# FrozenBurning/SceneDreamer

Hardware: NVIDIA H100
Metric: rendered Msamples/sec at 960x540x24spp (higher is better)
Workload: dtype f16x3 split (f32-grade), f32 accumulate; table/compositing f32

## Files before the change

scenedreamer_b200/csrc/render_fused.cu:

```cuda
#include <stdlib.h>

#include <map>
#include <mutex>
#include <utility>

#include "rf_common.cuh"

namespace rf {

int32_t *g_debug_buffer = nullptr;

struct Sample { float depth, nd; int idx; };

__device__ __forceinline__ Sample sample_at(const Params &p, const float *st, int row, int k, const float *frac,
                                            long long ray) {
    const float total = st[kStTotal * kRows + row];
    float r0, r1;
    if (p.uniforms == nullptr) {
        r0 = __fmul_rn(frac[k], total);
        r1 = __fmul_rn(frac[k + 1], total);
    } else {
        const float ns = (float)(p.S + 1);
        const bool any = total > 0.0f;
        const float u0 = any ? __ldg(p.uniforms + ray * (p.S + 1) + k) : 0.0f;
// ... 180 lines not shown
            h[q] = __byte_perm(a, b, 0x7632);
            const float la = v[2 * q] - __uint_as_float(a & 0xFFFF0000u);
            const float lb = v[2 * q + 1] - __uint_as_float(b & 0xFFFF0000u);
            l[q] = tc05::pack2<true>(la, lb);
        }
    } else {
#pragma unroll
        for (int q = 0; q < 4; q++) { h[q] = tc05::pack2<false>(v[2 * q], v[2 * q + 1]); l[q] = 0; }
    }
    hi = make_uint4(h[0], h[1], h[2], h[3]);
    lo = make_uint4(l[0], l[1], l[2], l[3]);
}

template <int PREC> __device__ __forceinline__ uint32_t one16() { return PREC == 1 ? 0x3F80u : 0x3C00u; }

template <bool RAW5D, int GU, int PREC, class Rec>
__device__ __forceinline__ void encode_features(const Params &p, uint32_t mask, const float *sScale, int half, const float (&x)[5],
                                                bool oob, uint4 (&fh)[8], uint4 (&fl)[8], Rec &&rec) {
#pragma unroll
    for (int i = 0; i < 8; i++) {
        const int level = half + 2 * i;
        float res[8];
        if (oob) {
#pragma unroll
            for (int c = 0; c < 8; c++) res[c] = 0.0f;
        } else {
            encode_level<RAW5D, GU>(p.table + ((size_t)level << p.log2_T) * 8, mask, sScale[level], x, res);
        }
        split8<PREC>(res, fh[i], fl[i]);
        rec(level, res);
    }
}

__device__ __forceinline__ uint4 label_chunk(uint32_t label, int half, uint32_t one) {
    const int k = (int)label - 8 * half;
    const uint32_t v = (k >= 0 && k < 8) ? one << (16 * (k & 1)) : 0u, q = k >> 1;
    return make_uint4(q == 0 ? v : 0u, q == 1 ? v : 0u, q == 2 ? v : 0u, (q == 3 ? v : 0u) | (half == 1 ? one << 16 : 0u));
}

template <bool X3>
__device__ __forceinline__ void store_layer0(uint8_t *sHhi, uint8_t *sHlo, int row, int half, const uint4 (&fh)[8],
                                             const uint4 (&fl)[8], uint4 ext) {
#pragma unroll
    for (int i = 0; i < 8; i++) {
        const uint32_t off = tc05::chunk_off(kRows, row, half + 2 * i);
        *reinterpret_cast<uint4 *>(sHhi + off) = fh[i];
        if constexpr (X3) *reinterpret_cast<uint4 *>(sHlo + off) = fl[i];
    }
    const uint32_t off = tc05::chunk_off(kRows, row, kFeat / 8 + half);
    *reinterpret_cast<uint4 *>(sHhi + off) = ext;
    if constexpr (X3) *reinterpret_cast<uint4 *>(sHlo + off) = make_uint4(0, 0, 0, 0);
}

template <int PREC, bool RAW5D, int MODE, bool TRAIN, bool RAYQ = false, int GU = 8>
__global__ void __launch_bounds__(kThreads, 1)
mlp_kernel(const Params p)
{
    static_assert(!RAYQ || (MODE == kRender && !TRAIN && !RAW5D), "ray slots: inference render over the pre-blended table");
    constexpr bool SKY = MODE == kSky, BWD = MODE == kBwd || MODE == kSkyBwd, SKYBWD = MODE == kSkyBwd;
    constexpr bool ONE_STEP = SKY || SKYBWD;
    constexpr int NACT = Net<MODE>::NACT;
    static_assert(!TRAIN || ((MODE == kRender || MODE == kSky) && !RAW5D), "the training record is written by the forward networks");
    static_assert(!BWD || PREC == 1, "the gradient chains run in the range-safe bf16x3 mode");
    constexpr bool X3 = PREC != 0;
    constexpr bool BF16 = PREC == 1;
    constexpr Smem SM = smem_map();
    constexpr int PARTS = X3 ? 2 : 1;
    constexpr int NH = Net<MODE>::NH, NL = Net<MODE>::NL;
    static_assert(SM.total <= 232448, "shared memory map exceeds the 227 KB a CTA can have");
    static_assert(Net<MODE>::NBIAS <= Net<kRender>::NBIAS, "bias table slot");
    extern __shared__ __align__(1024) uint8_t smem[];
    uint8_t *sHhi = smem + SM.h_hi;
    uint8_t *sHlo = smem + SM.h_lo;
    uint8_t *sRing = smem + SM.ring;
    float *sF = reinterpret_cast<float *>(smem + SM.fsec);
    float *sBias = reinterpret_cast<float *>(smem + SM.bias);
    float *sScale = reinterpret_cast<float *>(smem + SM.scales);
    float *sFrac = reinterpret_cast<float *>(smem + SM.frac);
    float *sSig = reinterpret_cast<float *>(smem + SM.sig);
    float *sState = reinterpret_cast<float *>(smem + SM.state);
    uint64_t *bars = reinterpret_cast<uint64_t *>(smem + SM.bars);
    uint32_t *sWalk = reinterpret_cast<uint32_t *>(smem + SM.walk);
    constexpr uint32_t kSlot = 16384, kSlabB = 2048 * PARTS;
    constexpr int kSps = kSlot / kSlabB;
    constexpr int kStepStages = step_stages<MODE>(kSps);
    constexpr uint32_t kWalk0 = hand_plan<MODE>(0).walk, kWalkH = hand_plan<MODE>(1).walk, kWalkL = hand_plan<MODE>(NL - 1).walk;
    constexpr uint32_t kSrc0 = hand_plan<MODE>(0).src, kSrcH = hand_plan<MODE>(1).src, kSrcL = hand_plan<MODE>(NL - 1).src;
    static_assert(SKYBWD || hand_all_staged<MODE>(NL - 1), "the epilogue reads the last layer from the operand buffer only");
    constexpr bool ESTOP = MODE == kRender && !TRAIN;
    volatile int *sStop = reinterpret_cast<volatile int *>(smem + SM.stop);
    volatile int *sVote = sStop + 2;
    int *sVoted = const_cast<int *>(sStop) + 4;

    const int tid = threadIdx.x, warp = tid >> 5, lane = tid & 31;
    const int wmult = (MODE == kBwd && p.work_mult > 1) ? p.work_mult : 1;
    const int n_work = RAYQ ? (int)gridDim.x : (ONE_STEP ? p.n_tiles : *p.n_live * wmult);
    auto rec_work = [&](int work) {
        if constexpr (MODE != kBwd) return work;
        int first;
        asm volatile("ld.global.nc.s32 %0, [%1];" : "=r"(first) : "l"(p.view));
        return work + first * wmult;
    };
    constexpr bool STATE = MODE == kRender;
    const int S = ONE_STEP ? 1 : p.S;
    const int SL = RAYQ ? 0x3fffffff : S;
    uint4 *sInfo = reinterpret_cast<uint4 *>(sState + kStFloats * kRows);
    int *sDone = reinterpret_cast<int *>(sInfo + 4 * kRows);
    int2 *sCur = reinterpret_cast<int2 *>(sDone + 2 * kRows);
    volatile int *sExh = reinterpret_cast<volatile int *>(sCur + kRows);
    static_assert(4 * kRows * 16 + 2 * kRows * 4 + kRows * 8 + 32 <= kStFloats * kRows * 4, "ray-slot bookkeeping fits the second state buffer");

    if (tid == 0) {
        for (int i = 0; i < 4; i++) tc05::mbar_init(&bars[B_WFULL + i], 1);
        tc05::mbar_init(&bars[B_FEAT], kGatherThreads);
        tc05::mbar_init(&bars[B_HFREE], 1);
        for (int rb = 0; rb < 2; rb++) {
            tc05::mbar_init(&bars[B_OPND + rb], kEpiThreads / 2);
            tc05::mbar_init(&bars[B_ACC + rb], 1);
            tc05::mbar_init(&bars[B_OUTRDY + rb], 1);
            tc05::mbar_init(&bars[B_EPIDONE + rb], kEpiThreads / 2);
            tc05::mbar_init(&bars[B_EPIDONE + 2 + rb], kEpiThreads / 2);
        }
        for (int i = 0; i < 2; i++) { tc05::mbar_init(&bars[B_STRDY + i], kRows); tc05::mbar_init(&bars[B_STFREE + i], kEpiThreads); }
        tc05::mbar_init(&bars[B_COMP], kEpiThreads);
        for (int i = 0; i < 4; i++) tc05::mbar_init(&bars[B_WEMPTY + i], 4);
        tc05::fence_mbar_init();
        int k = 0;
        for (int l = 0; l < NL; l++) {
            const int nK = layerK<MODE>(l) / 16, ncb = layerN<MODE>(l) / 64, nsb = block_stages(nK, kSps);
            const uint32_t walk = l == 0 ? kWalk0 : (l == NL - 1 ? kWalkL : kWalkH);
            for (int rb = 0; rb < 2; rb++)
                for (int pos = 0; pos < ncb; pos++) {
                    const int c = (walk >> (8 * pos)) & 3u;
                    uint32_t po = (uint32_t)(layerOff<MODE>(l, PARTS) + (int64_t)c * nK * kSlabB);
                    for (int js = 0; js < nsb; js++) {
                        const uint32_t bytes = (uint32_t)stage_slabs(nK, kSps, js) * kSlabB;
                        sWalk[k++] = (po >> 11) | ((bytes >> 11) << 16);
                        po += bytes;
                    }
                }
        }
    }
    if (tid < 2) { sStop[tid] = RAYQ ? 0x7fffffff : kMaxS + 1; sVote[tid] = 0; sVoted[tid] = 0; }
    if constexpr (RAYQ) {
        for (int i = tid; i < kRows; i += kThreads) { sCur[i] = make_int2(-1, 0); sDone[i] = 0; sDone[kRows + i] = 0; }
        if (tid < 5) sExh[tid] = 0;
    }
    volatile int *sWork = reinterpret_cast<volatile int *>(smem + SM.sched);
    volatile int *sPub = sWork + 4;
    if (tid == 0) *sPub = 0;
    const bool dyn = STATE && !RAYQ && p.work_counter != nullptr;
    auto fetch_work = [&](int it) -> int {
        if (!dyn) {
            const int w = (int)blockIdx.x + it * (int)gridDim.x;
            return w < n_work ? w : -1;
        }
        while (*sPub <= it) {
        }
        return sWork[it & 3];
    };
    if (STATE) {
        for (int i = tid; i < kLevels; i += kThreads) sScale[i] = exp2f(i * p.level_S) * p.base_res - 1.0f;
        for (int i = tid; i <= p.S; i += kThreads) sFrac[i] = p.fractions[i];
    }
    __syncthreads();
    const uint32_t mask = SKY ? 0u : ((1u << p.log2_T) - 1u);

    if (warp < 8) {
        set_maxnreg<kRegsEpi>();
        const int row = tid & (kRows - 1), half = tid >> 7;
        const int rb = row >> 6;
        const bool rb_lead = (tid & 191) == 0;
        auto last_vote = [&](int s) {
            __threadfence_block();
            const bool last = atomicAdd(&sVoted[s & 1], 1) == 1;
            if (last) {
                sVoted[s & 1] = 0;
                __threadfence_block();
            }
            return last;
        };
        const float *acc_cta = p.acc + (size_t)blockIdx.x * 2 * kRows * kAccCols;
        uint32_t n = 0;
        int loaded_img = -1;
        for (int it = 0;; it++) {
            const int work = fetch_work(it);
            if (work < 0) break;
            const int tile = RAYQ ? 0 : (ONE_STEP ? work : p.tile_list[rec_work(work) / wmult]);
            const TileCoord tc = tile_coord(p, tile);
            const int buf = it & 1;
            const float *st = sState + buf * kStFloats * kRows;
            if (Net<MODE>::TAIL && loaded_img != tc.img) {
                const float *packF = reinterpret_cast<const float *>(p.pack + (long long)tc.img * p.pack_stride +
                                                                     layerOff<MODE>(NL, PARTS));
                asm volatile("bar.sync 1, 256;" ::: "memory");
                for (int i = tid; i < kFTotal; i += kEpiThreads) sF[i] = __ldg(packF + i);
                asm volatile("bar.sync 1, 256;" ::: "memory");
                loaded_img = tc.img;
            }
            const int y = tc.y0 + (row >> 4), x = tc.x0 + (row & 15);
            const bool in_img = (y < p.H) && (x < p.W);
            const long long ray = ((long long)tc.img * p.H + y) * p.W + x;
            uint32_t flags = in_img ? 4u : 0u, labs = 0;
            float dir0 = 0.0f, ori0 = 0.0f;
            if (STATE && !RAYQ) {
                tc05::mbar_wait(&bars[B_STRDY + buf], (it >> 1) & 1);
                flags = __float_as_uint(st[kStFlags * kRows + row]);
                labs = __float_as_uint(st[kStLab * kRows + row]);
                dir0 = st[(kStDir + 0) * kRows + row];
                ori0 = __ldg(p.cam_ori + tc.img * 3);
            }
            (void)labs;
            const bool live = flags & 1u, valid = flags & 4u;
            float outc[32];
#pragma unroll
            for (int c = 0; c < 32; c++) outc[c] = 0.0f;
            float Wsum = 0.0f, Dsum = 0.0f, Dcomp = 0.0f, Eexcl = 0.0f;
            bool is_gnd = false;
// ... 132 lines not shown
                stg_ld<32>(sHhi, sHlo, row, ccol, c);
                if constexpr (BWD) {
                    float c2[32];
                    stg_ld<32>(sHhi, sHlo, row, ccol + 32, c2);
                    tc05::mbar_arrive(&bars[B_EPIDONE + (go & 1u) * 2 + rb]);
                    if (rb_lead) SDB_STAMP(n, NH, 5 + 2 * rb);
                    float *dst = p.tr.dx0 + slot * kFeat + half * 64;
#pragma unroll
                    for (int q = 0; q < 4; q++) st_global_v8f(dst + 8 * q, &c[8 * q]);
#pragma unroll
                    for (int q = 0; q < 4; q++) st_global_v8f(dst + 32 + 8 * q, &c2[8 * q]);
                    continue;
                }
                tc05::mbar_arrive(&bars[B_EPIDONE + (go & 1u) * 2 + rb]);
                if (rb_lead) SDB_STAMP(n, NH, 5 + 2 * rb);
                if constexpr (SKY) {
#pragma unroll
                    for (int j = 0; j < 32; j++) outc[j] = c[j];
                } else if constexpr (RAYQ) {
                    tc05::named_sync(4 + rb, 128);
                    const float sigma = (sSig[row] + sSig[kRows + row]) + sF[kFBsig];
                    const uint4 info = sInfo[(s & 3) * kRows + row];
                    const int rq = (int)info.z;
                    const uint32_t code = info.w;
                    const int s_ray = (int)(code & 0xffu);
                    const bool act = rq >= 0 && rq != skip_ray;
                    if (act && (code & 0x100u)) {
#pragma unroll
                        for (int j = 0; j < 32; j++) outc[j] = 0.0f;
                        Wsum = 0.0f; Dsum = 0.0f; Dcomp = 0.0f; Eexcl = 0.0f;
                    }
                    float w = 0.0f;
                    bool fin = false;
                    if (act) {
                        const float depth = __uint_as_float(info.x), nd = __uint_as_float(info.y);
                        w = sample_weight(sigma, nd, p.dists_scale, Eexcl);
                        composite_add(w, depth, Wsum, Dsum, Dcomp);
                        if (half == 0 && p.weights_out) p.weights_out[(long long)rq * S + s_ray] = w;
                        fin = (code & 0x200u) || (p.early_T > 0.0f && expf(-Eexcl) < p.early_T);
                    }
                    colour_add(w, c, outc);
                    if (act && fin) {
                        const bool nosky = !(code & 0x800u) || (code & 0x1000u);
                        finish_ray(p, 0, rq, nosky, half * 32, outc, Wsum, __fadd_rn(Dsum, Dcomp), half == 0);
                        skip_ray = (code & 0x200u) ? -1 : rq;
                    }
                    if (half == 0) sDone[(s & 1) * kRows + row] = (act && fin && !(code & 0x200u)) ? rq + 1 : 0;
                    {
                        const bool idle = !act || fin;
                        const bool wall = __all_sync(0xffffffffu, idle);
                        if (lane == 0 && !wall) sVote[s & 1] = 1;
                        tc05::named_sync(4 + rb, 128);
                        if (rb_lead && last_vote(s)) {
                            if (sVote[s & 1] == 0 && sExh[s & 3] != 0 && sStop[0] > s + 2) sStop[0] = s + 2;
                            sVote[s & 1] = 0;
                        }
                    }
                    tc05::mbar_arrive(&bars[B_COMP]);
                } else {
                    tc05::named_sync(4 + rb, 128);
                    const float sigma = (sSig[row] + sSig[kRows + row]) + sF[kFBsig];
                    float w = sample_weight(sigma, sm.nd, p.dists_scale, Eexcl);
                    w = live ? w : 0.0f;
                    composite_add(w, sm.depth, Wsum, Dsum, Dcomp);
                    if constexpr (TRAIN) {
                        if (half == 0) { p.tr.sig[slot] = sigma; p.tr.nds[slot] = __fmul_rn(sm.nd, p.dists_scale); }
                        float *cd = p.tr.c + slot * kOutC + half * 32;
#pragma unroll
                        for (int q = 0; q < 4; q++) st_global_v8f(cd + 8 * q, &c[8 * q]);
                    }
                    if (half == 0 && valid) {
                        if (p.weights_out) p.weights_out[ray * S + s] = w;
                        if (p.rdepth_out) p.rdepth_out[ray * S + s] = sm.depth;
                    }
                    if (ESTOP && p.early_T > 0.0f) {
                        const bool done = !live || expf(-Eexcl) < p.early_T;
                        const bool wall = __all_sync(0xffffffffu, done);
                        if (lane == 0 && !wall) sVote[s & 1] = 1;
                        tc05::named_sync(4 + rb, 128);
                        if (rb_lead && last_vote(s)) {
                            if (sVote[s & 1] == 0 && sStop[buf] > S) sStop[buf] = s + 2;
                            sVote[s & 1] = 0;
                        }
                    }
                    colour_add(w, c, outc);
                }
            }
            if constexpr (SKY) {
                if (valid) {
                    float4 *dst = reinterpret_cast<float4 *>(p.sky_out + ray * kOutC + half * 32);
#pragma unroll
                    for (int q = 0; q < 8; q++) dst[q] = make_float4(outc[4 * q], outc[4 * q + 1], outc[4 * q + 2], outc[4 * q + 3]);
                }
                float *red = sSig;
                asm volatile("bar.sync 1, 256;" ::: "memory");
#pragma unroll
                for (int j = 0; j < 32; j++) {
                    float v = valid ? outc[j] : 0.0f;
#pragma unroll
                    for (int o = 16; o > 0; o >>= 1) v += __shfl_xor_sync(0xffffffffu, v, o);
                    if (lane == 0) red[(warp & 3) * kOutC + half * 32 + j] = v;
                }
                asm volatile("bar.sync 1, 256;" ::: "memory");
                if (tid < kOutC)
                    p.sky_partial[(long long)tile * kOutC + tid] =
                        (red[tid] + red[kOutC + tid]) + (red[2 * kOutC + tid] + red[3 * kOutC + tid]);
            } else if constexpr (RAYQ) {
// ... 41 lines not shown
          }
          for (int s = 0; s < SL; s++, n++) {
              if (ESTOP && s >= 2 && s >= sStop[it & 1]) break;
#pragma unroll 1
              for (int l = 0; l < NL; l++) {
                  const uint32_t g = n * NL + l, buf = g & 1u;
                  const int N = layerN<MODE>(l), nK = layerK<MODE>(l) / 16;
                  const int ncb = N / 64, nsb = block_stages(nK, kSps), ns0 = group0_stages(nK, kSps);
#pragma unroll 1
                  for (int rb = 0; rb < 2; rb++) {
                      if (t == 0) SDB_MARK(2, 1, n, l);
                      if (g >= 2) tc05::mbar_wait(&bars[B_EPIDONE + buf * 2 + rb], ((g >> 1) - 1) & 1);
                      if (l == 0) {
                          if (rb == 0) tc05::mbar_wait(&bars[B_FEAT], n & 1);
                      } else {
                          tc05::mbar_wait(&bars[B_OPND + rb], (n * NH + l - 1) & 1);
                      }
                      if (t == 0) SDB_MARK(2, 2, n, l);
                      if (t == 0) SDB_STAMP(n, l, 2 * rb);
                      TSplit ts;
                      ts.start();
                      const uint32_t dst = (blockIdx.x * 2 + buf) * kRows * kAccCols + acc_off(rb * 64, 0);
                      const uint32_t walk = l == 0 ? kWalk0 : (l == NL - 1 ? kWalkL : kWalkH);
                      float x[32], y[32];
                      auto issue = [&](float (&d)[32], int js0, int js1) {
                          for (int js = js0; js < js1; js++) {
                              const uint32_t slot = q & 3u;
                              tc05::mbar_wait(&bars[B_WFULL + slot], (q >> 2) & 1u);
                              ts.lap(kSplitFull);
                              const uint32_t sb = tc05::smem_u32(sRing + slot * kSlot);
                              const int kk0 = stage_slab0(nK, kSps, js), ns = stage_slabs(nK, kSps, js);
                              tc05::wgmma_fence();
#pragma unroll
                              for (int i = 0; i < kSps; i++) {
                                  if (i >= ns) break;
                                  const uint32_t aoff = (uint32_t)(kk0 + i) * 2 * kLboA + rb * 1024;
                                  const uint64_t ah = tc05::make_smem_desc(tc05::smem_u32(sHhi) + aoff, kLboA, kSbo);
                                  const uint64_t bh = tc05::make_smem_desc(sb + i * kSlabB, 1024, kSbo);
                                  tc05::wgmma_m64n64k16<BF16, 0, 0>(d, ah, bh, (js > js0 || i > 0) ? 1u : 0u);
                                  if constexpr (X3) {
                                      const uint64_t al = tc05::make_smem_desc(tc05::smem_u32(sHlo) + aoff, kLboA, kSbo);
                                      tc05::wgmma_m64n64k16<BF16, 0, 0>(d, al, bh, 1u);
                                      tc05::wgmma_m64n64k16<BF16, 0, 0>(d, ah, bh + (2048 >> 4), 1u);
                                  }
                              }
                              tc05::wgmma_commit();
                              q++;
                              ts.lap(kSplitIssue);
                          }
                      };
                      auto retire = [&](int pending) {
                          auto release = [&]() {
                              ts.lap(kSplitWait);
                              if (lane == 0) tc05::mbar_arrive(&bars[B_WEMPTY + (qr & 3u)]);
                              qr++;
                              ts.lap(kSplitRelease);
                          };
#pragma unroll 1
                          for (int k = pending - 1; k > 0; k--) {
                              tc05::wgmma_wait_n(k);
                              release();
                          }
                          tc05::wgmma_wait<0>();
                          if (pending > 0) release();
                      };
                      bool g0_done = false;
                      auto block = [&](float (&a)[32], float (&b)[32], int pos) {
                          const uint32_t w = walk >> (8 * pos);
                          const int c = (int)(w & 3u);
                          issue(b, ns0, nsb);
                          retire(g0_done ? nsb - ns0 : nsb);
                          g0_done = false;
                          tc05::wgmma_fence_acc(a);
                          tc05::wgmma_fence_acc(b);
                          if (nsb > ns0) {
#pragma unroll
                              for (int i = 0; i < 32; i++) a[i] = __fadd_rn(a[i], b[i]);
                          }
                          uint32_t ft;
                          asm volatile("mov.u32 %0, %%tid.x;" : "=r"(ft));
                          ft -= kMmaWarp0 * 32;
                          if (BIAS && l > 0) {
                              const float *bias = sBias + (l - 1) * kHidden + c * 64;
#pragma unroll
                              for (int i = 0; i < 32; i += 2) {
                                  const float2 bb = *reinterpret_cast<const float2 *>(bias + tc05::frag_col(ft, i));
                                  a[i] = __fadd_rn(a[i], bb.x);
                                  a[i + 1] = __fadd_rn(a[i + 1], bb.y);
                              }
                          }
                          ts.lap(kSplitReduce);
                          if (pos + 1 < ncb) issue(b, 0, ns0);
                          if (!(w & kHStaged)) {
#ifndef SDB_AB_NO_ACC
                              float *out = p.acc + (dst + (uint32_t)(c & 1) * 4096u + acc_off(tc05::frag_row(ft, 0), tc05::frag_col(ft, 0)));
#pragma unroll
                              for (int i = 0; i < 32; i += 2)
                                  *reinterpret_cast<float2 *>(out + (i >> 2) * 128 + ((i >> 1) & 1) * 32) = make_float2(a[i], a[i + 1]);
#endif
                          } else {
                              if (w & kHDelayed) {
                                  retire(ns0);
                                  g0_done = true;
                              }
                              if (l == 0 && (w & kHFirst) && g >= 1)
                                  tc05::mbar_wait(&bars[B_EPIDONE + ((g - 1) & 1u) * 2 + rb], ((g - 1) >> 1) & 1u);
                              if (w & kHBarrier) tc05::named_sync(3, 128);
// ... 207 lines not shown
                if (half == 0) {
                    const RayVoxels vox = ray_state(p, st, row, tc.img, pix, valid);
                    const uint32_t flags = (valid && vox.first != 0 ? 1u : 0u) | (vox.last == 0 ? 2u : 0u) | (valid ? 4u : 0u);
                    st[kStFlags * kRows + row] = __uint_as_float(flags);
                }
                asm volatile("bar.sync 2, 256;" ::: "memory");
                if (half == 0) tc05::mbar_arrive(&bars[B_STRDY + buf]);
                const bool live = __float_as_uint(st[kStFlags * kRows + row]) & 1u;
                const uint32_t labs = __float_as_uint(st[kStLab * kRows + row]);
                const float dir[3] = {st[(kStDir + 0) * kRows + row], st[(kStDir + 1) * kRows + row], st[(kStDir + 2) * kRows + row]};
                const float ori[3] = {__ldg(p.cam_ori + tc.img * 3 + 0), __ldg(p.cam_ori + tc.img * 3 + 1), __ldg(p.cam_ori + tc.img * 3 + 2)};
                float x5[5];
                x5[3] = __fmul_rn(__fadd_rn(__ldg(p.genc + tc.img * 2 + 0), 1.0f), 0.5f);
                x5[4] = __fmul_rn(__fadd_rn(__ldg(p.genc + tc.img * 2 + 1), 1.0f), 0.5f);

                for (int s = 0; s < S; s++, n++) {
                    uint4 fh[8], fl[8];
                    const Sample sm = sample_at(p, st, row, s, sFrac, ray);
                    const bool outside = grid_coord(p, dir, ori, sm.depth, x5);
                    const bool oob = !live || outside;
                    const uint32_t label = (labs >> (4 * sm.idx)) & 15u;
                    if constexpr (TRAIN) {
                        const long long slot = ((long long)work * S + s) * kRows + row;
                        if (half == 0) p.tr.x3[slot] = make_float4(x5[0], x5[1], x5[2], oob ? -1.0f : 1.0f);
                        *reinterpret_cast<uint4 *>(rec_chunk(p.tr.x0, slot, kX0Cols / 8, kFeat / 8 + half)) = label_chunk(label, half, one16<1>());
                    }
                    encode_features<RAW5D, 8, PREC>(p, mask, sScale, half, x5, oob, fh, fl, [&](int level, const float (&res)[8]) {
                        if constexpr (TRAIN) {
                            const long long slot = ((long long)work * S + s) * kRows + row;
                            *reinterpret_cast<uint4 *>(rec_chunk(p.tr.x0, slot, kX0Cols / 8, level)) =
                                make_uint4(tc05::pack2<true>(res[0], res[1]), tc05::pack2<true>(res[2], res[3]),
                                           tc05::pack2<true>(res[4], res[5]), tc05::pack2<true>(res[6], res[7]));
                        }
                    });
                    const uint4 ext = label_chunk(label, half, one16<PREC>());
                    if (gt == 0) SDB_MARK(4, 3, n, it);
                    if (n > 0) tc05::mbar_wait_backoff(&bars[B_HFREE], (n - 1) & 1);
                    if (gt == 0) SDB_MARK(4, 4, n, it);
                    if (ESTOP && s >= 2 && s >= sStop[buf]) break;
                    store_layer0<X3>(sHhi, sHlo, row, half, fh, fl, ext);
                    tc05::fence_proxy_async_smem();
                    tc05::mbar_arrive(&bars[B_FEAT]);
                }
            }
        }
    } else {
        set_maxnreg<kRegsProd>();
        if (warp == kProducerWarp0 && elect_one()) {
            uint32_t n = 0, q = 0;
            uint32_t waited = 0;
            auto wait_empty = [&]() {
                if (q < 4) return;
                const uint32_t c = SDB_CLOCK();
                tc05::mbar_wait(&bars[B_WEMPTY + (q & 3u)], ((q >> 2) - 1) & 1u);
                waited += SDB_CLOCK() - c;
            };
            for (int it = 0;; it++) {
                const int work = fetch_work(it);
                if (work < 0) break;
                const int tile = RAYQ ? 0 : (ONE_STEP ? work : p.tile_list[rec_work(work) / wmult]);
                const uint8_t *pack = p.pack + (long long)tile_coord(p, tile).img * p.pack_stride;
                for (int s = 0; s < SL; s++, n++) {
                    SDB_MARK(3, 1, n, it);
                    waited = 0;
                    wait_empty();
                    if (ESTOP && s >= 2 && s >= sStop[it & 1]) break;
                    for (int k = 0; k < kStepStages; k++, q++) {
                        if (k > 0) wait_empty();
                        const uint32_t e = sWalk[k], bytes = (e >> 16) << 11, slot = q & 3u;
                        tc05::mbar_arrive_expect_tx(&bars[B_WFULL + slot], bytes);
                        tc05::bulk_g2s(sRing + slot * kSlot, pack + ((e & 0xffffu) << 11), bytes, &bars[B_WFULL + slot]);
                    }
                    SDB_STAMP_PROD(n, waited);
                }
            }
        }
    }
}

__device__ __forceinline__ void sky_only_ray(const Params &p, int img, long long ray) {
    const bool is_gnd = __ldg(p.cam_ori + img * 3) <= 1.0f;
    const float none[kOutC] = {};
    finish_ray(p, img, ray, is_gnd, 0, none, 0.0f, 0.0f, true);
    for (int s = 0; s < p.S; s++) {
        if (p.weights_out) p.weights_out[ray * p.S + s] = 0.0f;
        if (p.rdepth_out) p.rdepth_out[ray * p.S + s] = 0.0f;
    }
}

__global__ void __launch_bounds__(kRows)
prepass_kernel(const Params p, int32_t *tile_list, int32_t *n_live)
{
    const int tile = blockIdx.x, row = threadIdx.x;
    const TileCoord tc = tile_coord(p, tile);
    const int y = tc.y0 + (row >> 4), x = tc.x0 + (row & 15);
    const bool valid = (y < p.H) && (x < p.W);
    const long long ray = ((long long)tc.img * p.H + y) * p.W + x;
    const bool live = valid && (__ldg(p.voxel_id + ray * p.M) != 0);
    const int any = __syncthreads_or(live ? 1 : 0);
    if (any) {
        if (row == 0) {
            const int w = atomicAdd(n_live, 1);
            tile_list[w] = tile;
            if (p.tr.tile_work) p.tr.tile_work[tile] = w;
        }
        return;
    }
    if (row == 0 && p.tr.tile_work) p.tr.tile_work[tile] = -1;
    if (valid) sky_only_ray(p, tc.img, ray);
}

__global__ void __launch_bounds__(kRows)
train_prepass_kernel(const Params p, int32_t *hdr)
{
    const int tile = blockIdx.x, row = threadIdx.x;
    const TileCoord tc = tile_coord(p, tile);
    const int y = tc.y0 + (row >> 4), x = tc.x0 + (row & 15);
    const bool valid = (y < p.H) && (x < p.W);
    const long long ray = ((long long)tc.img * p.H + y) * p.W + x;
    const bool live = valid && (__ldg(p.voxel_id + ray * p.M) != 0);
    if (__syncthreads_or(live ? 1 : 0)) {
        if (row == 0) p.tr.tile_work[tile] = atomicAdd(hdr + 2 + 2 * tc.img, 1);
        return;
    }
    if (row == 0) p.tr.tile_work[tile] = -1;
    if (valid) sky_only_ray(p, tc.img, ray);
}

__global__ void __launch_bounds__(256)
train_list_kernel(const Params p, int32_t *hdr, int32_t *tile_list)
// ... 158 lines not shown
            float *F = reinterpret_cast<float *>(pack + layerOff<MODE>(NL, PARTS));
            float v = 0.0f;
            if (u < kHidden) v = wsig[u];
            else if (u == kFBsig) v = bsig[0];
            F[u] = v;
            return;
        }
        u -= kFTotal;
    }
    if (u >= Net<MODE>::NBIAS) return;
    const int l = 1 + (int)(u / kHidden), nn = (int)(u % kHidden);
    const float v = l == NL - 1 ? bout[nn] : bh[(long long)(l - 1) * kHidden + nn];
    reinterpret_cast<float *>(pack + biasOff<MODE>(PARTS))[u] = packed_value<PREC>(v);
}

template <bool SKY>
int launch_pack(const float *w0, const float *b0, const float *emb, int n_labels, const float *wh, const float *bh,
                const float *wsig, const float *bsig, const float *wout, const float *bout, int precision, void *pack,
                cudaStream_t st) {
    constexpr int MODE = SKY ? kSky : kRender;
    long long n = (SKY ? 0 : kFTotal) + Net<MODE>::NBIAS;
    for (int l = 0; l < Net<MODE>::NL; l++) n += (long long)layerK<MODE>(l) * layerN<MODE>(l);
    const int blocks = (int)((n + 255) / 256);
    if (precision == 1)
        pack_kernel<1, SKY><<<blocks, 256, 0, st>>>(w0, b0, emb, n_labels, wh, bh, wsig, bsig, wout, bout, (uint8_t *)pack);
    else if (precision == 2)
        pack_kernel<2, SKY><<<blocks, 256, 0, st>>>(w0, b0, emb, n_labels, wh, bh, wsig, bsig, wout, bout, (uint8_t *)pack);
    else
        pack_kernel<0, SKY><<<blocks, 256, 0, st>>>(w0, b0, emb, n_labels, wh, bh, wsig, bsig, wout, bout, (uint8_t *)pack);
    SDB_CHECK_LAUNCH();
    return SDB_OK;
}

static int acc_buffers(int grid, cudaStream_t st, float **out) {
    static std::mutex mu;
    static std::map<std::pair<int, cudaStream_t>, std::pair<float *, int>> bufs;
    int dev = 0;
    SDB_CUDA(cudaGetDevice(&dev));
    std::lock_guard<std::mutex> lk(mu);
    std::pair<float *, int> &b = bufs[std::make_pair(dev, st)];
    if (b.second < grid) {
        cudaStreamCaptureStatus cs = cudaStreamCaptureStatusNone;
        SDB_CUDA(cudaStreamIsCapturing(st, &cs));
        if (cs != cudaStreamCaptureStatusNone) return SDB_EUNSUPPORTED;
        if (b.first) SDB_CUDA(cudaFree(b.first));
        b = std::make_pair((float *)nullptr, 0);
        SDB_CUDA(cudaMalloc(&b.first, (size_t)grid * 2 * kRows * kAccCols * sizeof(float)));
        b.second = grid;
    }
    *out = b.first;
    return SDB_OK;
}

template <int PREC, bool RAW5D, int MODE, bool TRAIN = false, bool RAYQ = false, int GU = 8>
int launch_mlp(const Params &p_in, int grid, cudaStream_t st) {
    Params p = p_in;
    const int e = acc_buffers(grid, st, &p.acc);
    if (e != SDB_OK) return e;
    const size_t smem = smem_map().total;
    cudaFuncAttributes fa;
    SDB_CUDA(cudaFuncGetAttributes(&fa, mlp_kernel<PREC, RAW5D, MODE, TRAIN, RAYQ, GU>));
    if (fa.numRegs < kRegsLaunch) return SDB_EUNSUPPORTED;
    SDB_CUDA(cudaFuncSetAttribute(mlp_kernel<PREC, RAW5D, MODE, TRAIN, RAYQ, GU>, cudaFuncAttributeMaxDynamicSharedMemorySize, (int)smem));
    mlp_kernel<PREC, RAW5D, MODE, TRAIN, RAYQ, GU><<<grid, kThreads, smem, st>>>(p);
    SDB_CHECK_LAUNCH();
    return SDB_OK;
}

int launch_train_forward(const Params &p, int precision, int grid, cudaStream_t st) {
    return precision == 0 ? launch_mlp<0, false, kRender, true>(p, grid, st) : launch_mlp<2, false, kRender, true>(p, grid, st);
}
int launch_bwd_chain(const Params &p, int grid, cudaStream_t st) { return launch_mlp<1, false, kBwd>(p, grid, st); }
int launch_sky_train_forward(const Params &p, int grid, cudaStream_t st) { return launch_mlp<2, false, kSky, true>(p, grid, st); }
int launch_sky_bwd_chain(const Params &p, int grid, cudaStream_t st) { return launch_mlp<1, false, kSkyBwd>(p, grid, st); }
int launch_train_prepass(const Params &p, int32_t *hdr, int32_t *tile_list, cudaStream_t st) {
    SDB_CUDA(cudaMemsetAsync(hdr, 0, (size_t)(1 + 2 * p.n_img) * 4, st));
    train_prepass_kernel<<<p.n_tiles, kRows, 0, st>>>(p, hdr);
    SDB_CHECK_LAUNCH();
    train_list_kernel<<<(p.n_tiles + 255) / 256, 256, 0, st>>>(p, hdr, tile_list);
    SDB_CHECK_LAUNCH();
    return SDB_OK;
}
int launch_prepass(const Params &p, int32_t *ws, cudaStream_t st) {
    SDB_CUDA(cudaMemsetAsync(ws, 0, 16, st));
    prepass_kernel<<<p.n_tiles, kRows, 0, st>>>(p, ws + 4, ws);
    SDB_CHECK_LAUNCH();
    return SDB_OK;
}

template <int MODE>
__global__ void __launch_bounds__(256)
pack_bwd_kernel(const float *w1, const float *wh, const float *wsig, const float *wout, uint8_t *pack)
{
    constexpr int PARTS = 2, NL = Net<MODE>::NL;
    const long long t = blockIdx.x * (long long)blockDim.x + threadIdx.x;
    long long nW = 0;
    for (int l = 0; l < NL; l++) nW += (long long)layerK<MODE>(l) * layerN<MODE>(l);
    if (t < nW) {
        long long r = t;
        int l = 0;
        while (r >= (long long)layerK<MODE>(l) * layerN<MODE>(l)) { r -= (long long)layerK<MODE>(l) * layerN<MODE>(l); l++; }
        const int K = layerK<MODE>(l);
        const int nn = (int)(r / K), k = (int)(r % K);
        float v;
        if (l == 0) v = wout[(long long)k * kHidden + nn];
        else if (MODE == kBwd && l == NL - 1) v = w1[(long long)k * kFeat + nn];
        else v = wh[((long long)((MODE == kBwd ? 5 : 4) - l) * kHidden + k) * kHidden + nn];
        uint8_t *base = pack + layerOff<MODE>(l, PARTS);
        const __nv_bfloat16 hi = __float2bfloat16_rn(v);
        const __nv_bfloat16 lo = __float2bfloat16_rn(v - __bfloat162float(hi));
        *reinterpret_cast<__nv_bfloat16 *>(base + wpack_off(K / 16, PARTS, nn, k, 0)) = hi;
        *reinterpret_cast<__nv_bfloat16 *>(base + wpack_off(K / 16, PARTS, nn, k, 1)) = lo;
        return;
    }
    if (!Net<MODE>::TAIL) return;
    const long long u = t - nW;
    if (u >= kFTotal) return;
    float *F = reinterpret_cast<float *>(pack + layerOff<MODE>(NL, PARTS));
    F[u] = u < kHidden ? wsig[u] : 0.0f;
// ... 168 lines not shown
    p.sample_depth = sp->sample_depth; p.dists_scale = sp->dists_scale;
    p.early_T = sp->early_stop_transmittance > 0.0f ? sp->early_stop_transmittance : 0.0f;
    p.fractions = sp->d_fractions; p.uniforms = sp->d_uniforms;
    p.lut = sp->d_label_lut; p.n_lut = sp->n_lut;
    p.raw5d = sp->d_table != nullptr;
    p.table = p.raw5d ? sp->d_table : sp->d_table3;
    p.log2_T = sp->log2_T; p.level_S = sp->level_S; p.base_res = sp->base_res;
    p.pack = (const uint8_t *)sp->d_mlp_pack; p.pack_stride = sp->mlp_pack_stride;
    p.sky = sp->d_sky; p.sky_avg = sp->d_sky_avg;
    p.net_out = sp->d_net_out; p.depth_out = sp->d_depth_out; p.total_weight = sp->d_total_weight;
    p.weights_out = sp->d_weights_out; p.rdepth_out = sp->d_rand_depth_out;
    p.debug = g_debug_buffer;
    p.tiles_x = sdb_div_up(p.W, kTileW); p.tiles_y = sdb_div_up(p.H, kTileH);
    p.n_tiles = p.n_img * p.tiles_x * p.tiles_y;
    if (!sp->d_cam_ori) p.cam_ori = reinterpret_cast<const float *>((const int32_t *)sp->d_workspace + 4 + p.n_tiles);
    return SDB_OK;
}

int stage_cam_ori(const sdb_render_params *sp, const Params &p, cudaStream_t st)
{
    if (sp->d_cam_ori) return SDB_OK;
    set_cam_kernel<<<1, 1, 0, st>>>(const_cast<float *>(p.cam_ori), sp->cam_ori_value[0], sp->cam_ori_value[1], sp->cam_ori_value[2]);
    SDB_CHECK_LAUNCH();
    return SDB_OK;
}
}

extern "C" int sdb_render_rays_forward(const sdb_render_params *sp, void *stream)
{
    using namespace rf;
    cudaStream_t st = (cudaStream_t)stream;
    Params p;
    {
        const int rc = params_from_abi(sp, p);
        if (rc != SDB_OK) return rc;
    }
    int32_t *ws = (int32_t *)sp->d_workspace;
    p.n_live = ws; p.tile_list = ws + 4; p.steps_done = ws + 1; p.work_counter = ws + 2;
    {
        const int rc = stage_cam_ori(sp, p, st);
        if (rc != SDB_OK) return rc;
    }
    const char *env_rq = getenv("SDB_RAY_SLOTS");
    const bool rayq = !p.raw5d && p.n_img == 1 && !(env_rq && atoi(env_rq) == 0);
    if (rayq) {
        int32_t *ray_list = ws + 8 + p.n_tiles;
        SDB_CUDA(cudaMemsetAsync(ws, 0, 16, st));
        prepass_rays_kernel<<<p.n_tiles, kRows, 0, st>>>(p, ray_list, ws);
        SDB_CHECK_LAUNCH();
        p.tile_list = ray_list;
        const long long groups = ((long long)p.H * p.W + kRows - 1) / kRows;
        const int grid = groups < sdb_num_sms() ? (int)groups : sdb_num_sms();
        int rc;
        if (sp->precision == 0) rc = launch_mlp<0, false, kRender, false, true>(p, grid, st);
        else if (sp->precision == 1) rc = launch_mlp<1, false, kRender, false, true>(p, grid, st);
        else {
            static const int gu = [] { const char *e = getenv("SDB_GATHER_UNROLL"); return e ? atoi(e) : 2; }();
            if (gu == 8) rc = launch_mlp<2, false, kRender, false, true>(p, grid, st);
            else rc = launch_mlp<2, false, kRender, false, true, 2>(p, grid, st);
        }
        if (rc != SDB_OK) return rc;
        set_flag_kernel<<<1, 1, 0, st>>>(ws + 3);
        SDB_CHECK_LAUNCH();
        return SDB_OK;
    }
    {
        const int rc = launch_prepass(p, ws, st);
        if (rc != SDB_OK) return rc;
    }
    const int grid = p.n_tiles < sdb_num_sms() ? p.n_tiles : sdb_num_sms();
    switch (sp->precision * 2 + (p.raw5d ? 1 : 0)) {
        case 0: return launch_mlp<0, false, kRender>(p, grid, st);
        case 1: return launch_mlp<0, true, kRender>(p, grid, st);
        case 2: return launch_mlp<1, false, kRender>(p, grid, st);
        case 3: return launch_mlp<1, true, kRender>(p, grid, st);
        case 4: return launch_mlp<2, false, kRender>(p, grid, st);
        default: return launch_mlp<2, true, kRender>(p, grid, st);
    }
}
```

scenedreamer_b200/csrc/tc05.cuh:

```cuda
#pragma once
#include <cuda_bf16.h>
#include <cuda_fp16.h>
#include <stdint.h>

namespace tc05 {

__device__ __forceinline__ uint32_t smem_u32(const void *p) {
    return (uint32_t)__cvta_generic_to_shared(p);
}

__device__ __forceinline__ uint64_t make_smem_desc(uint32_t saddr, uint32_t lbo_bytes, uint32_t sbo_bytes) {
    uint64_t d = 0;
    d |= (uint64_t)((saddr & 0x3FFFF) >> 4);
    d |= (uint64_t)((lbo_bytes >> 4) & 0x3FFF) << 16;
    d |= (uint64_t)((sbo_bytes >> 4) & 0x3FFF) << 32;
    return d;
}

template <bool BF16, int TA, int TB>
__device__ __forceinline__ void wgmma_m64n16k16(float (&d)[8], uint64_t da, uint64_t db, uint32_t accumulate) {
    if constexpr (BF16)
        asm volatile("{\n\t.reg .pred p;\n\tsetp.ne.b32 p, %10, 0;\n\t"
                     "wgmma.mma_async.sync.aligned.m64n16k16.f32.bf16.bf16 {%0, %1, %2, %3, %4, %5, %6, %7}, %8, %9, p, 1, 1, %11, %12;\n\t}\n"
                     : "+f"(d[0]), "+f"(d[1]), "+f"(d[2]), "+f"(d[3]), "+f"(d[4]), "+f"(d[5]), "+f"(d[6]), "+f"(d[7])
// ... 50 lines not shown
#pragma unroll
    for (int i = 0; i < R; i++) asm volatile("" : "+f"(d[i])::"memory");
}
__device__ __forceinline__ void st_shared_v2f(uint32_t saddr, float a, float b) {
    asm volatile("st.shared.v2.f32 [%0], {%1, %2};" ::"r"(saddr), "f"(a), "f"(b) : "memory");
}
__device__ __forceinline__ void fence_proxy_async_smem() { asm volatile("fence.proxy.async.shared::cta;" ::: "memory"); }

__device__ __forceinline__ void named_sync(uint32_t id, uint32_t threads) {
    asm volatile("bar.sync %0, %1;" ::"r"(id), "r"(threads) : "memory");
}

__device__ __forceinline__ int frag_row(int t, int i) { return ((t >> 5) << 4) + ((t & 31) >> 2) + (((i >> 1) & 1) << 3); }
__device__ __forceinline__ int frag_col(int t, int i) { return ((i >> 2) << 3) + ((t & 3) << 1) + (i & 1); }

__device__ __forceinline__ void mbar_init(uint64_t *bar, uint32_t count) {
    asm volatile("mbarrier.init.shared::cta.b64 [%0], %1;" ::"r"(smem_u32(bar)), "r"(count) : "memory");
}
__device__ __forceinline__ void fence_mbar_init() { asm volatile("fence.mbarrier_init.release.cluster;" ::: "memory"); }
__device__ __forceinline__ void mbar_arrive(uint64_t *bar) {
    asm volatile("mbarrier.arrive.shared::cta.b64 _, [%0];" ::"r"(smem_u32(bar)) : "memory");
}
__device__ __forceinline__ void mbar_arrive_expect_tx(uint64_t *bar, uint32_t bytes) {
    asm volatile("mbarrier.arrive.expect_tx.shared::cta.b64 _, [%0], %1;" ::"r"(smem_u32(bar)), "r"(bytes) : "memory");
}
__device__ __forceinline__ bool mbar_try_wait(uint64_t *bar, uint32_t parity) {
    uint32_t ok;
    asm volatile(
        "{\n\t"
        ".reg .pred p;\n\t"
        "mbarrier.try_wait.parity.shared::cta.b64 p, [%1], %2;\n\t"
        "selp.b32 %0, 1, 0, p;\n\t"
        "}\n"
        : "=r"(ok)
        : "r"(smem_u32(bar)), "r"(parity)
        : "memory");
    return ok != 0;
}
__device__ __forceinline__ void mbar_wait(uint64_t *bar, uint32_t parity) {
    while (!mbar_try_wait(bar, parity)) {
    }
}
__device__ __forceinline__ void mbar_wait_backoff(uint64_t *bar, uint32_t parity, uint32_t ns = 256) {
    while (!mbar_try_wait(bar, parity)) __nanosleep(ns);
}

__device__ __forceinline__ void bulk_g2s(void *dst_smem, const void *src_gmem, uint32_t bytes, uint64_t *bar) {
    asm volatile("cp.async.bulk.shared::cluster.global.mbarrier::complete_tx::bytes [%0], [%1], %2, [%3];" ::"r"(
                     smem_u32(dst_smem)),
                 "l"(src_gmem), "r"(bytes), "r"(smem_u32(bar))
                 : "memory");
}

template <bool BF16>
__device__ __forceinline__ uint32_t pack2(float a, float b) {
    if constexpr (BF16) {
        __nv_bfloat162 v = __floats2bfloat162_rn(a, b);
        return *reinterpret_cast<uint32_t *>(&v);
    } else {
        __half2 v = __floats2half2_rn(a, b);
        return *reinterpret_cast<uint32_t *>(&v);
    }
}
template <bool BF16>
__device__ __forceinline__ float2 unpack2(uint32_t u) {
    if constexpr (BF16) {
        return __bfloat1622float2(*reinterpret_cast<__nv_bfloat162 *>(&u));
    } else {
        return __half22float2(*reinterpret_cast<__half2 *>(&u));
    }
}

__host__ __device__ __forceinline__ constexpr uint32_t chunk_off(uint32_t rows, uint32_t r, uint32_t kc) {
    return kc * rows * 16u + (r >> 3) * 128u + (r & 7u) * 16u;
}

}
```

Baseline: 401.6.

## Pair ray-slot CTAs in clusters and multicast weight slabs across the pair

Launches the ray-slot render kernel as 2-CTA clusters. Each CTA fetches half of every weight stage and multicasts it into both CTAs' rings, which halves per-CTA global/L2 weight traffic. The ring-empty barrier now waits for consumers in both CTAs, and the early-stop vote is exchanged between partners so both stop at the same step. The cost is a lockstep coupling between paired CTAs (a slow partner stalls the other), cluster sync overhead, and possibly fewer resident CTAs if cluster occupancy limits the grid.

```diff
diff --git a/scenedreamer_b200/csrc/render_fused.cu b/scenedreamer_b200/csrc/render_fused.cu
--- a/scenedreamer_b200/csrc/render_fused.cu
+++ b/scenedreamer_b200/csrc/render_fused.cu
@@ -256,11 +256,12 @@
     if constexpr (X3) *reinterpret_cast<uint4 *>(sHlo + off) = make_uint4(0, 0, 0, 0);
 }
 
-template <int PREC, bool RAW5D, int MODE, bool TRAIN, bool RAYQ = false, int GU = 8>
+template <int PREC, bool RAW5D, int MODE, bool TRAIN, bool RAYQ = false, int GU = 8, bool PAIR = false>
 __global__ void __launch_bounds__(kThreads, 1)
 mlp_kernel(const Params p)
 {
     static_assert(!RAYQ || (MODE == kRender && !TRAIN && !RAW5D), "ray slots: inference render over the pre-blended table");
+    static_assert(!PAIR || RAYQ, "CTA pairs: the ray-slot kernel only (one open-ended work item per CTA)");
     constexpr bool SKY = MODE == kSky, BWD = MODE == kBwd || MODE == kSkyBwd, SKYBWD = MODE == kSkyBwd;
     constexpr bool ONE_STEP = SKY || SKYBWD;
     constexpr int NACT = Net<MODE>::NACT;
@@ -295,6 +296,8 @@
     volatile int *sStop = reinterpret_cast<volatile int *>(smem + SM.stop);
     volatile int *sVote = sStop + 2;
     int *sVoted = const_cast<int *>(sStop) + 4;
+    int *sPairVote = const_cast<int *>(sStop) + 6;
+    auto partner = []() { return tc05::cluster_ctarank() ^ 1u; };
 
     const int tid = threadIdx.x, warp = tid >> 5, lane = tid & 31;
     const int wmult = (MODE == kBwd && p.work_mult > 1) ? p.work_mult : 1;
@@ -327,7 +330,7 @@
         }
         for (int i = 0; i < 2; i++) { tc05::mbar_init(&bars[B_STRDY + i], kRows); tc05::mbar_init(&bars[B_STFREE + i], kEpiThreads); }
         tc05::mbar_init(&bars[B_COMP], kEpiThreads);
-        for (int i = 0; i < 4; i++) tc05::mbar_init(&bars[B_WEMPTY + i], 4);
+        for (int i = 0; i < 4; i++) tc05::mbar_init(&bars[B_WEMPTY + i], PAIR ? 8 : 4);
         tc05::fence_mbar_init();
         int k = 0;
         for (int l = 0; l < NL; l++) {
@@ -345,7 +348,7 @@
                 }
         }
     }
-    if (tid < 2) { sStop[tid] = RAYQ ? 0x7fffffff : kMaxS + 1; sVote[tid] = 0; sVoted[tid] = 0; }
+    if (tid < 2) { sStop[tid] = RAYQ ? 0x7fffffff : kMaxS + 1; sVote[tid] = 0; sVoted[tid] = 0; if (PAIR) sPairVote[tid] = 0; }
     if constexpr (RAYQ) {
         for (int i = tid; i < kRows; i += kThreads) { sCur[i] = make_int2(-1, 0); sDone[i] = 0; sDone[kRows + i] = 0; }
         if (tid < 5) sExh[tid] = 0;
@@ -367,7 +370,8 @@
         for (int i = tid; i < kLevels; i += kThreads) sScale[i] = exp2f(i * p.level_S) * p.base_res - 1.0f;
         for (int i = tid; i <= p.S; i += kThreads) sFrac[i] = p.fractions[i];
     }
-    __syncthreads();
+    if constexpr (PAIR) tc05::cluster_sync();
+    else __syncthreads();
     const uint32_t mask = SKY ? 0u : ((1u << p.log2_T) - 1u);
 
     if (warp < 8) {
@@ -606,7 +610,15 @@
                         if (lane == 0 && !wall) sVote[s & 1] = 1;
                         tc05::named_sync(4 + rb, 128);
                         if (rb_lead && last_vote(s)) {
-                            if (sVote[s & 1] == 0 && sExh[s & 3] != 0 && sStop[0] > s + 2) sStop[0] = s + 2;
+                            bool stop = sVote[s & 1] == 0 && sExh[s & 3] != 0;
+                            if constexpr (PAIR) {
+                                tc05::st_release_cluster(tc05::mapa(&sPairVote[s & 1], partner()), (uint32_t)(s + 1) << 1 | (stop ? 1u : 0u));
+                                uint32_t v;
+                                do v = tc05::ld_acquire_cluster(&sPairVote[s & 1]);
+                                while ((v >> 1) != (uint32_t)(s + 1));
+                                stop = stop && (v & 1u);
+                            }
+                            if (stop && sStop[0] > s + 2) sStop[0] = s + 2;
                             sVote[s & 1] = 0;
                         }
                     }
@@ -754,7 +766,10 @@
                       auto retire = [&](int pending) {
                           auto release = [&]() {
                               ts.lap(kSplitWait);
-                              if (lane == 0) tc05::mbar_arrive(&bars[B_WEMPTY + (qr & 3u)]);
+                              if (lane == 0) {
+                                  tc05::mbar_arrive(&bars[B_WEMPTY + (qr & 3u)]);
+                                  if constexpr (PAIR) tc05::mbar_arrive_remote(tc05::mapa(&bars[B_WEMPTY + (qr & 3u)], partner()));
+                              }
                               qr++;
                               ts.lap(kSplitRelease);
                           };
@@ -1068,7 +1083,8 @@
             auto wait_empty = [&]() {
                 if (q < 4) return;
                 const uint32_t c = SDB_CLOCK();
-                tc05::mbar_wait(&bars[B_WEMPTY + (q & 3u)], ((q >> 2) - 1) & 1u);
+                if constexpr (PAIR) tc05::mbar_wait_cluster(&bars[B_WEMPTY + (q & 3u)], ((q >> 2) - 1) & 1u);
+                else tc05::mbar_wait(&bars[B_WEMPTY + (q & 3u)], ((q >> 2) - 1) & 1u);
                 waited += SDB_CLOCK() - c;
             };
             for (int it = 0;; it++) {
@@ -1085,13 +1101,20 @@
                         if (k > 0) wait_empty();
                         const uint32_t e = sWalk[k], bytes = (e >> 16) << 11, slot = q & 3u;
                         tc05::mbar_arrive_expect_tx(&bars[B_WFULL + slot], bytes);
-                        tc05::bulk_g2s(sRing + slot * kSlot, pack + ((e & 0xffffu) << 11), bytes, &bars[B_WFULL + slot]);
+                        if constexpr (PAIR) {
+                            const uint32_t h = bytes >> 1, o = tc05::cluster_ctarank() * h;
+                            tc05::bulk_g2s_multicast(sRing + slot * kSlot + o, pack + ((e & 0xffffu) << 11) + o, h,
+                                                     &bars[B_WFULL + slot], 0x3);
+                        } else {
+                            tc05::bulk_g2s(sRing + slot * kSlot, pack + ((e & 0xffffu) << 11), bytes, &bars[B_WFULL + slot]);
+                        }
                     }
                     SDB_STAMP_PROD(n, waited);
                 }
             }
         }
     }
+    if constexpr (PAIR) tc05::cluster_sync();
 }
 
 __device__ __forceinline__ void sky_only_ray(const Params &p, int img, long long ray) {
@@ -1356,19 +1379,51 @@
     return SDB_OK;
 }
 
-template <int PREC, bool RAW5D, int MODE, bool TRAIN = false, bool RAYQ = false, int GU = 8>
+static cudaLaunchConfig_t pair_config(int grid, size_t smem, cudaStream_t st, cudaLaunchAttribute &cl) {
+    cl.id = cudaLaunchAttributeClusterDimension;
+    cl.val.clusterDim.x = 2; cl.val.clusterDim.y = 1; cl.val.clusterDim.z = 1;
+    cudaLaunchConfig_t cfg = {};
+    cfg.gridDim = dim3(grid); cfg.blockDim = dim3(kThreads); cfg.dynamicSmemBytes = smem; cfg.stream = st;
+    cfg.attrs = &cl; cfg.numAttrs = 1;
+    return cfg;
+}
+
+template <int PREC, bool RAW5D, int MODE, bool TRAIN = false, bool RAYQ = false, int GU = 8, bool PAIR = false>
 int launch_mlp(const Params &p_in, int grid, cudaStream_t st) {
     Params p = p_in;
     const int e = acc_buffers(grid, st, &p.acc);
     if (e != SDB_OK) return e;
     const size_t smem = smem_map().total;
     cudaFuncAttributes fa;
-    SDB_CUDA(cudaFuncGetAttributes(&fa, mlp_kernel<PREC, RAW5D, MODE, TRAIN, RAYQ, GU>));
+    SDB_CUDA(cudaFuncGetAttributes(&fa, mlp_kernel<PREC, RAW5D, MODE, TRAIN, RAYQ, GU, PAIR>));
     if (fa.numRegs < kRegsLaunch) return SDB_EUNSUPPORTED;
-    SDB_CUDA(cudaFuncSetAttribute(mlp_kernel<PREC, RAW5D, MODE, TRAIN, RAYQ, GU>, cudaFuncAttributeMaxDynamicSharedMemorySize, (int)smem));
-    mlp_kernel<PREC, RAW5D, MODE, TRAIN, RAYQ, GU><<<grid, kThreads, smem, st>>>(p);
+    SDB_CUDA(cudaFuncSetAttribute(mlp_kernel<PREC, RAW5D, MODE, TRAIN, RAYQ, GU, PAIR>, cudaFuncAttributeMaxDynamicSharedMemorySize, (int)smem));
+    if constexpr (PAIR) {
+        cudaLaunchAttribute cl;
+        const cudaLaunchConfig_t cfg = pair_config(grid, smem, st, cl);
+        SDB_CUDA(cudaLaunchKernelEx(&cfg, mlp_kernel<PREC, RAW5D, MODE, TRAIN, RAYQ, GU, PAIR>, p));
+    } else {
+        mlp_kernel<PREC, RAW5D, MODE, TRAIN, RAYQ, GU><<<grid, kThreads, smem, st>>>(p);
+    }
     SDB_CHECK_LAUNCH();
     return SDB_OK;
+}
+
+template <int PREC, int GU>
+int launch_ray_slots(const Params &p, int grid, cudaStream_t st) {
+    const char *env = getenv("SDB_RAYSLOT_PAIRS");
+    if (grid >= 2 && !(env && atoi(env) == 0)) {
+        auto kern = mlp_kernel<PREC, false, kRender, false, true, GU, true>;
+        const size_t smem = smem_map().total;
+        SDB_CUDA(cudaFuncSetAttribute(kern, cudaFuncAttributeMaxDynamicSharedMemorySize, (int)smem));
+        cudaLaunchAttribute cl;
+        const cudaLaunchConfig_t cfg = pair_config(grid / 2 * 2, smem, st, cl);
+        int clusters = 0;
+        SDB_CUDA(cudaOccupancyMaxActiveClusters(&clusters, kern, &cfg));
+        const int pairs = clusters < grid / 2 ? clusters : grid / 2;
+        if (pairs >= 1) return launch_mlp<PREC, false, kRender, false, true, GU, true>(p, 2 * pairs, st);
+    }
+    return launch_mlp<PREC, false, kRender, false, true, GU>(p, grid, st);
 }
 
 int launch_train_forward(const Params &p, int precision, int grid, cudaStream_t st) {
@@ -1643,12 +1698,12 @@
         const long long groups = ((long long)p.H * p.W + kRows - 1) / kRows;
         const int grid = groups < sdb_num_sms() ? (int)groups : sdb_num_sms();
         int rc;
-        if (sp->precision == 0) rc = launch_mlp<0, false, kRender, false, true>(p, grid, st);
-        else if (sp->precision == 1) rc = launch_mlp<1, false, kRender, false, true>(p, grid, st);
+        if (sp->precision == 0) rc = launch_ray_slots<0, 8>(p, grid, st);
+        else if (sp->precision == 1) rc = launch_ray_slots<1, 8>(p, grid, st);
         else {
             static const int gu = [] { const char *e = getenv("SDB_GATHER_UNROLL"); return e ? atoi(e) : 2; }();
-            if (gu == 8) rc = launch_mlp<2, false, kRender, false, true>(p, grid, st);
-            else rc = launch_mlp<2, false, kRender, false, true, 2>(p, grid, st);
+            if (gu == 8) rc = launch_ray_slots<2, 8>(p, grid, st);
+            else rc = launch_ray_slots<2, 2>(p, grid, st);
         }
         if (rc != SDB_OK) return rc;
         set_flag_kernel<<<1, 1, 0, st>>>(ws + 3);
diff --git a/scenedreamer_b200/csrc/tc05.cuh b/scenedreamer_b200/csrc/tc05.cuh
--- a/scenedreamer_b200/csrc/tc05.cuh
+++ b/scenedreamer_b200/csrc/tc05.cuh
@@ -126,6 +126,52 @@
                  : "memory");
 }
 
+__device__ __forceinline__ uint32_t cluster_ctarank() {
+    uint32_t r;
+    asm volatile("mov.u32 %0, %%cluster_ctarank;" : "=r"(r));
+    return r;
+}
+__device__ __forceinline__ uint32_t mapa(const void *p, uint32_t rank) {
+    uint32_t a;
+    asm volatile("mapa.shared::cluster.u32 %0, %1, %2;" : "=r"(a) : "r"(smem_u32(p)), "r"(rank));
+    return a;
+}
+__device__ __forceinline__ void mbar_arrive_remote(uint32_t remote) {
+    asm volatile("mbarrier.arrive.release.cluster.shared::cluster.b64 _, [%0];" ::"r"(remote) : "memory");
+}
+__device__ __forceinline__ void mbar_wait_cluster(uint64_t *bar, uint32_t parity) {
+    uint32_t ok = 0;
+    while (!ok)
+        asm volatile(
+            "{\n\t"
+            ".reg .pred p;\n\t"
+            "mbarrier.try_wait.parity.acquire.cluster.shared::cta.b64 p, [%1], %2;\n\t"
+            "selp.b32 %0, 1, 0, p;\n\t"
+            "}\n"
+            : "=r"(ok)
+            : "r"(smem_u32(bar)), "r"(parity)
+            : "memory");
+}
+__device__ __forceinline__ void st_release_cluster(uint32_t remote, uint32_t v) {
+    asm volatile("st.release.cluster.shared::cluster.u32 [%0], %1;" ::"r"(remote), "r"(v) : "memory");
+}
+__device__ __forceinline__ uint32_t ld_acquire_cluster(const void *p) {
+    uint32_t v;
+    asm volatile("ld.acquire.cluster.shared::cta.u32 %0, [%1];" : "=r"(v) : "r"(smem_u32(p)) : "memory");
+    return v;
+}
+__device__ __forceinline__ void cluster_sync() {
+    asm volatile("barrier.cluster.arrive.release;\n\tbarrier.cluster.wait.acquire;" ::: "memory");
+}
+__device__ __forceinline__ void bulk_g2s_multicast(void *dst_smem, const void *src_gmem, uint32_t bytes, uint64_t *bar,
+                                                   uint16_t cta_mask) {
+    asm volatile(
+        "cp.async.bulk.shared::cluster.global.mbarrier::complete_tx::bytes.multicast::cluster [%0], [%1], %2, [%3], %4;" ::"r"(
+            smem_u32(dst_smem)),
+        "l"(src_gmem), "r"(bytes), "r"(smem_u32(bar)), "h"(cta_mask)
+        : "memory");
+}
+
 template <bool BF16>
 __device__ __forceinline__ uint32_t pack2(float a, float b) {
     if constexpr (BF16) {
```

After: 228.8, median of 6. 43.0% lower.
